# LLNL/ppo_and_friends

Measured on AMD Instinct MI355X. Metric: env_steps_per_sec, higher is better.
Workload: dtype f32; 1 GPU; C2 CartPole-v1 MLP (4->128x3->2 actor, ->1 critic), envs_per_proc=4096, ts_per_rollout=128, fixed-length synthetic trajectories, batch_size=256, epochs_per_iter=10; parallelism=dp1, hip_graphs=True

## Files before the change

### ppo_and_friends_amd/csrc/ppo_update_dev.hpp

```cpp
#pragma once
#include "action_heads.hpp"
#include "wgrad_tile.hpp"
#include <cstddef>
#include <cstring>

namespace ppoaf {

struct WsDev {
    float* hbuf[2];
    float* dbuf[2];
    float* outpart[2];
    float* xbuf[2];
    int W;
    int xcc[2];
    int Bp;
};

struct UpdateDev {
    NetDev net[2];
    const float* params; float* grads; float* exp_avg; float* exp_avg_sq; float* slabs;
    long bucket_total;
    int64_t* step_counts; const float* lr; double* norm_scratch;
    float beta1, beta2, adam_eps, grad_scale, max_norm; int head_kind;
    const float* obs; const float* critic_obs; const void* raw_actions;
    const float* adv; const float* old_lp; const float* rtg; float* values;
    const int64_t* perm; const int32_t* row_map; long n_rows;
    int64_t* cursor; long B, batch_stride, mb_offset, cursor_advance;
    int normalize_values, n_ranks;
    float* vn_mean; float* vn_var; double* vn_count; const double* vn_records;
    const double* adv_records;
    int normalize_adv, use_huber, pregathered;
    float surr_clip, entropy_weight, kl_loss_weight, huber_delta, min_std;
    float* loss_partials; double* totals;
    int n_wg;
    int confine;
    int split;
    WsDev sp;
    int n_slices; int slices[8];
};

inline long ws_seg_off(const NetDev& n) {
    const long szW0 = ((long)n.H * n.in_dim + 3) & ~3L;
    return n.depth == 0 ? 0 : szW0 + n.H + (long)(n.depth - 1) * ((long)n.H * n.H + n.H);
}
inline long ws_seg_len(const NetDev& n) { return n.size - ws_seg_off(n); }

inline int split_wgrad_jobs(const NetDev& n) {
    const int t = n.H / 16, t2 = (t + 1) / 2, p0 = ((n.in_dim + 15) / 16 + 1) / 2;
    return (n.depth - 1) * t * t2 + t * p0 + 1;
}
inline int split_wgrad_per_xcd(const UpdateDev& u) { return (split_wgrad_jobs(u.net[0]) + split_wgrad_jobs(u.net[1]) + 7) / 8; }
inline int split_wgrad_blocks(const UpdateDev& u) { return 8 * split_wgrad_per_xcd(u); }

inline size_t ws_layout(const UpdateDev& u, WsDev* ws, char* base) {
    const long Bp = (u.B + 63) & ~63L;
    size_t off = 0;
    auto take = [&](size_t floats) { const size_t o = off; off += (floats * 4 + 255) & ~(size_t)255; return o; };
    for (int w = 0; w < 2; ++w) {
        const NetDev& n = u.net[w];
        const size_t plane = (size_t)n.depth * Bp * n.H;
        const size_t oh = take(plane), od = take(plane), oo = take((size_t)((u.B + 15) / 16) * ws_seg_len(n));
        const size_t ox = take((size_t)Bp * 64);
        if (ws) {
            ws->hbuf[w] = reinterpret_cast<float*>(base + oh);
            ws->dbuf[w] = reinterpret_cast<float*>(base + od);
            ws->outpart[w] = reinterpret_cast<float*>(base + oo);
            ws->xbuf[w] = reinterpret_cast<float*>(base + ox);
        }
    }
    if (ws) ws->Bp = (int)Bp;
    return off;
}

constexpr int kPairHeaderBytes = 256;
constexpr int kPairRecBytes = 16 * 1024;
constexpr int kPairMaxTiles = 32;
constexpr long long kPairWaitTicks = 200000000LL;

struct PairDev {
    unsigned char* base;
    long net_off[2];
};

inline bool pair_eligible(const NetDev& n) { return n.H == 256 && n.depth >= 2 && n.depth <= 4; }
inline int pair_phases(const NetDev& n) { return 2 * n.depth - 3; }
inline size_t pair_region_offset(const UpdateDev& u) {
    UpdateDev f = u;
    if (u.batch_stride > f.B) f.B = u.batch_stride;
    return ws_layout(f, nullptr, nullptr);
}
inline size_t pair_region_layout(const UpdateDev& u, PairDev* p, char* region) {
    size_t off = kPairHeaderBytes;
    for (int w = 0; w < 2; ++w) {
        const bool on = pair_eligible(u.net[w]);
        if (p) p->net_off[w] = on ? (long)off : 0;
        if (on) off += (size_t)pair_phases(u.net[w]) * kPairMaxTiles * 2 * kPairRecBytes;
    }
    if (p) p->base = reinterpret_cast<unsigned char*>(region);
    return off;
}

constexpr int kWgradThreads = 256;

struct SplitJob {
    int l, ot, itile;
    bool two;
    long ldw;
    long off_w, off_b;
};
template <int H>
__device__ __forceinline__ long split_off_w(const NetDev& nd, const int l) {
    const long szW0 = ((long)H * nd.in_dim + 3) & ~3L;
    return l == 0 ? 0 : szW0 + H + (long)(l - 1) * ((long)H * H + H);
}
template <int H>
__device__ __forceinline__ bool split_job_decode(const UpdateDev& u, const int which, const int job, SplitJob& sj) {
    const auto& nd = u.net[which];
    const int in_dim = nd.in_dim, depth = nd.depth;
    constexpr int t = H / 16, t2 = (t + 1) / 2;
    const int n_it0 = (in_dim + 15) / 16, p0 = (n_it0 + 1) / 2;
    const int n_hidden = (depth - 1) * t * t2, n_l0 = t * p0;
    if (job >= n_hidden + n_l0) return false;
    int n_it;
    if (job < n_hidden) { sj.l = 1 + job / (t * t2); const int jj = job % (t * t2); sj.ot = jj / t2; sj.itile = 2 * (jj % t2); n_it = t; }
    else { sj.l = 0; const int jj = job - n_hidden; sj.ot = jj / p0; sj.itile = 2 * (jj % p0); n_it = n_it0; }
    const int l = sj.l;
    sj.two = sj.itile + 1 < n_it;
    sj.ldw = l >= 1 ? H : in_dim;
    sj.off_w = split_off_w<H>(nd, l);
    sj.off_b = l == 0 ? (((long)H * in_dim + 3) & ~3L)
                      : sj.off_w + (l < depth ? (long)H * H : (((long)nd.out_dim * H + 3) & ~3L));
    return true;
}
template <int H> __device__ __forceinline__ __amdgpu_buffer_rsrc_t split_panel_d(const UpdateDev& u, const int which, const int l) {
    return wgrad_rsrc(u.sp.dbuf[which] + (long)l * ((long)u.sp.Bp * H));
}
template <int H> __device__ __forceinline__ __amdgpu_buffer_rsrc_t split_panel_x(const UpdateDev& u, const int which, const int l) {
    return wgrad_rsrc(l >= 1 ? u.sp.hbuf[which] + (long)(l - 1) * ((long)u.sp.Bp * H) : u.sp.xbuf[which]);
}
__device__ __forceinline__ float split_out_fold(const float* outpart, const int n_hb, const long seg_len, const long idx) {
    float acc = 0.f;
    for (int g0 = 0; g0 < n_hb; g0 += 8) {
        float pv[8];
#pragma unroll
        for (int k = 0; k < 8; ++k) pv[k] = outpart[(long)(g0 + k < n_hb ? g0 + k : 0) * seg_len + idx];
#pragma unroll
        for (int k = 0; k < 8; ++k) if (g0 + k < n_hb) acc += pv[k];
    }
    return acc;
}

__device__ __forceinline__ void ppo_update_bookkeeping_totals(const UpdateDev& u) {
    const int lane = threadIdx.x;
    float p0 = 0.f, p2 = 0.f, p3 = 0.f, p4 = 0.f, p7 = 0.f;
    for (int g = lane; g < u.n_wg; g += 64) {
        const float* a = u.loss_partials + (long)g * 8;
        const float* cc = u.loss_partials + ((long)u.n_wg + g) * 8;
        p0 += a[0]; p3 += a[3]; p4 += a[4]; p7 += a[7]; p2 += cc[2];
    }
    p0 = wave_sum(p0); p2 = wave_sum(p2); p3 = wave_sum(p3); p4 = wave_sum(p4); p7 = wave_sum(p7);
    if (lane == 0) {
        const float n = (float)u.B;
        const float surr = p0 / n, ent = p3 / n, kl = p4 / n, crit = p2 / n;
        float total = surr;
        if (u.entropy_weight != 0.0f) total -= u.entropy_weight * ent;
        if (u.kl_loss_weight > 0.0f) total += u.kl_loss_weight * kl;
        u.totals[0] += (double)surr; u.totals[1] += (double)total; u.totals[2] += (double)crit;
        u.totals[3] += (double)ent; u.totals[4] += (double)kl;
        u.totals[5] += (double)u.loss_partials[5]; u.totals[6] += (double)u.loss_partials[6];
        u.totals[7] += p7 > 0.f ? 1.0 : 0.0;
        u.totals[8] += 1.0;
    }
}
__device__ __forceinline__ void ppo_update_bookkeeping_steps(const UpdateDev& u) {
    const int lane = threadIdx.x;
    if (lane < 2) {
        const int w = lane;
        const int64_t t = u.step_counts[w] + 1;
        u.step_counts[w] = t;
        u.norm_scratch[2 + 2 * w] = 1.0 - pow((double)u.beta1, (double)t);
        u.norm_scratch[3 + 2 * w] = sqrt(1.0 - pow((double)u.beta2, (double)t));
    }
}

__device__ __forceinline__ void ppo_update_bookkeeping_split(const UpdateDev& u) {
    if (threadIdx.x >= 64) return;
    ppo_update_bookkeeping_totals(u);
    ppo_update_bookkeeping_steps(u);
}

int make_update_dev(const ppoaf_ppo_update_args_t* a, UpdateDev& u);

inline ppoaf_ppo_update_args_t copy_update_args(const ppoaf_ppo_update_args_t* args) {
    ppoaf_ppo_update_args_t a;
    std::memset(&a, 0, sizeof(a));
    std::memcpy(&a, args, offsetof(ppoaf_ppo_update_args_t, n_action_slices));
    if (args->head_kind == PPOAF_HEAD_MULTI_CATEGORICAL) {
        a.n_action_slices = args->n_action_slices;
        std::memcpy(a.action_slices, args->action_slices, sizeof(a.action_slices));
    }
    return a;
}

__device__ __forceinline__ unsigned hw_xcc_id() {
    unsigned v;
    asm volatile("s_getreg_b32 %0, hwreg(HW_REG_XCC_ID)" : "=s"(v));
    return v & 0xfu;
}

template <bool NT, typename U>
__device__ __forceinline__ void ppo_head_loss(const U& u, const int which, const int g, const int out_dim,
                                              const float* __restrict__ log_std_p, const int* sRow,
                                              const float* sRowF, const float* sMisc, float* sActF, float* sOut,
                                              float* sDOut, const int lane, const long B) {
    const int s = lane;
    const int row = s < kRows ? sRow[s] : -1;
    const bool live = row >= 0;
    const float inv_B = 1.0f / (float)B;
    float part[8] = {0, 0, 0, 0, 0, 0, 0, 0};
    if (which == 0) {
        float logp = 0.f, ent = 0.f;
        float av = 0.f, lpo = 0.f;
        if (live) {
            av = sRowF[s]; lpo = sRowF[16 + s];
            if (u.normalize_adv) av = (av - sMisc[0]) / (sMisc[1] + 1e-8f);
        }
        if (u.head_kind == PPOAF_HEAD_CATEGORICAL) {
            const int s4 = lane >> 2, q = lane & 3;
            const bool live4 = sRow[s4] >= 0;
            float av4 = 0.f, lpo4 = 0.f;
            if (live4) {
                av4 = sRowF[s4]; lpo4 = sRowF[16 + s4];
                if (u.normalize_adv) av4 = (av4 - sMisc[0]) / (sMisc[1] + 1e-8f);
            }
            auto rsum = [](float v) { return group4_sum(v); };
            auto rmax = [](float v) { return group4_max(v); };
            const int k0 = q, k1 = q + 4;
            const bool v0 = k0 < out_dim, v1 = k1 < out_dim;
            const float z0 = v0 ? sOut[s4 * kMaxOut + k0] : -INFINITY, z1 = v1 ? sOut[s4 * kMaxOut + k1] : -INFINITY;
            const float m = rmax(fmaxf(z0, z1));
            float p0 = v0 ? expf(z0 - m) : 0.f, p1 = v1 ? expf(z1 - m) : 0.f;
            const float inv = 1.0f / rsum(p0 + p1);
            p0 *= inv; p1 *= inv;
            const float s2 = rsum(p0 + p1);
            int a = reinterpret_cast<const int*>(sActF)[s4 * 8];
            a = a < 0 ? 0 : (a >= out_dim ? out_dim - 1 : a);
            const float n0 = p0 / s2, n1 = p1 / s2;
            const float l0 = v0 ? logf(clamp_prob_u(n0)) : 0.f, l1 = v1 ? logf(clamp_prob_u(n1)) : 0.f;
            const float ent4 = -rsum((v0 ? n0 * l0 : 0.f) + (v1 ? n1 * l1 : 0.f));
            const float logp4 = rsum((k0 == a ? l0 : 0.f) + (k1 == a ? l1 : 0.f));
            const float ratio = expf(logp4 - lpo4);
            const float bad4 = (isnan(ratio) || isinf(ratio)) ? 1.f : 0.f;
            const float lo = 1.0f - u.surr_clip, hi = 1.0f + u.surr_clip;
            const float surr1 = ratio * av4, surr2 = fminf(fmaxf(ratio, lo), hi) * av4;
            float glp;
            if (surr1 <= surr2) glp = -av4 * ratio;
            else glp = (ratio >= lo && ratio <= hi) ? -av4 * ratio : 0.f;
            glp *= inv_B;
            const float gH = (u.entropy_weight != 0.0f) ? -u.entropy_weight * inv_B : 0.f;
            auto gk_of = [&](bool valid, int k, float nk, float lg) {
                if (!valid) return 0.f;
                const float ck = clamp_prob_u(nk);
                const float in_range = (nk >= FLT_EPSILON && nk <= 1.0f - FLT_EPSILON) ? 1.f : 0.f;
                float gk = gH * (-lg - nk * in_range / ck);
                if (k == a) gk += glp * in_range / ck;
                return gk;
            };
            float g0 = gk_of(v0, k0, n0, l0), g1 = gk_of(v1, k1, n1, l1);
            const float dot = rsum(g0 * n0 + g1 * n1);
            g0 = (g0 - dot) / s2; g1 = (g1 - dot) / s2;
            const float dot2 = rsum(g0 * p0 + g1 * p1);
            if (live4) {
                if (k0 < 8) sDOut[s4 * kMaxOut + k0] = p0 * (g0 - dot2);
                sDOut[s4 * kMaxOut + k1] = p1 * (g1 - dot2);
            } else {
                sDOut[s4 * kMaxOut + k0] = 0.f; sDOut[s4 * kMaxOut + k1] = 0.f;
                if (q == 0) for (int k2 = 8; k2 < kMaxOut; ++k2) sDOut[s4 * kMaxOut + k2] = 0.f;
            }
            const int src = (lane & 15) * 4;
            const float r_surr = __shfl(-fminf(surr1, surr2), src, 64), r_ent = __shfl(ent4, src, 64);
            const float r_kl = __shfl(lpo4 - logp4, src, 64), r_bad = __shfl(bad4, src, 64);
            if (live) { part[0] = r_surr; part[3] = r_ent; part[4] = r_kl; part[7] = r_bad; }
        } else if (u.head_kind >= PPOAF_HEAD_MULTI_CATEGORICAL) {
            if (live) {
                float z[8], dz[8];
#pragma unroll
                for (int k = 0; k < 8; ++k) z[k] = k < out_dim ? sOut[s * kMaxOut + k] : 0.f;
                const bool mcat = u.head_kind == PPOAF_HEAD_MULTI_CATEGORICAL;
                const float* x = sActF + s * 8;
                float p[8], sm[8];
                unsigned first = 0u, pick = 0u;
                if (mcat) {
                    first = mcat_starts(u.n_slices, u.slices);
                    mcat_probs(z, first, out_dim, p, sm);
                    pick = mcat_pick(reinterpret_cast<const int*>(x), u.n_slices, u.slices);
                    logp = mcat_logp(p, sm, pick);
                } else {
                    logp = bern_logp(z, x, out_dim);
                }
                const float ratio = expf(logp - lpo);
                if (isnan(ratio) || isinf(ratio)) part[7] = 1.f;
                const float lo = 1.0f - u.surr_clip, hi = 1.0f + u.surr_clip;
                const float surr1 = ratio * av, surr2 = fminf(fmaxf(ratio, lo), hi) * av;
                float glp;
                if (surr1 <= surr2) glp = -av * ratio;
                else glp = (ratio >= lo && ratio <= hi) ? -av * ratio : 0.f;
                glp *= inv_B;
                const float gH = (u.entropy_weight != 0.0f) ? -u.entropy_weight * inv_B : 0.f;
                ent = mcat ? mcat_entropy_grad(p, sm, first, pick, out_dim, glp, gH, dz)
                           : bern_entropy_grad(z, x, out_dim, glp, gH, dz);
                part[0] = -fminf(surr1, surr2);
                part[3] = ent;
                part[4] = lpo - logp;
#pragma unroll
                for (int k = 0; k < 8; ++k) sDOut[s * kMaxOut + k] = dz[k];
            } else if (s < kRows) {
                for (int k = 0; k < kMaxOut; ++k) sDOut[s * kMaxOut + k] = 0.f;
            }
        } else if (live) {
            const float* log_std = log_std_p;
            const float* x = sActF + s * 8;
            float lp = 0.f, slog = 0.f;
            ent = 0.f;
            for (int d = 0; d < out_dim; ++d) {
                const float sd = fmaxf(softplus_u(ld1<NT>(log_std + d)), u.min_std);
                const float mu = sOut[s * kMaxOut + d];
                const float zz = x[d] - mu;
                const float l0 = -logf(sd) - 0.91893853320467274178f;
                float l = -(zz * zz) / (2.0f * sd * sd) + l0;
                l = fminf(fmaxf(l, -100.f), 100.f);
                lp += l;
                const float th = tanhf(x[d]);
                slog += logf(fmaxf(1.0f - th * th, 1e-6f));
                const float thm = tanhf(mu);
                ent += logf(fmaxf(1.0f - thm * thm, 1e-6f)) - fminf(fmaxf(l0, -100.f), 100.f);
            }
            logp = lp - slog;
            const float ratio = expf(logp - lpo);
            if (isnan(ratio) || isinf(ratio)) part[7] = 1.f;
            const float lo = 1.0f - u.surr_clip, hi = 1.0f + u.surr_clip;
            const float surr1 = ratio * av, surr2 = fminf(fmaxf(ratio, lo), hi) * av;
            part[0] = -fminf(surr1, surr2);
            part[3] = ent;
            part[4] = lpo - logp;
            float glp;
            if (surr1 <= surr2) glp = -av * ratio;
            else glp = (ratio >= lo && ratio <= hi) ? -av * ratio : 0.f;
            glp *= inv_B;
            const float gH = (u.entropy_weight != 0.0f) ? -u.entropy_weight * inv_B : 0.f;
            for (int d = 0; d < out_dim; ++d) {
                const float ls = ld1<NT>(log_std + d);
                const float sp = softplus_u(ls), sd = fmaxf(sp, u.min_std);
                const float mu = sOut[s * kMaxOut + d];
                const float zz = x[d] - mu;
                const float l0 = -logf(sd) - 0.91893853320467274178f;
                const float l = -(zz * zz) / (2.0f * sd * sd) + l0;
                const float pass = (l >= -100.f && l <= 100.f) ? 1.f : 0.f;
                const float pass0 = (l0 >= -100.f && l0 <= 100.f) ? 1.f : 0.f;
                const float thm = tanhf(mu);
                const float pass_t = (1.0f - thm * thm >= 1e-6f) ? 1.f : 0.f;
                sDOut[s * kMaxOut + d] = glp * pass * zz / (sd * sd) - gH * pass_t * 2.0f * thm;
                if (d == 0) for (int k2 = out_dim; k2 < 8; ++k2) sDOut[s * kMaxOut + k2] = 0.f;
                const float dmax = sp > u.min_std ? 1.f : (sp == u.min_std ? 0.5f : 0.f);
                const float dsp = ls > 20.f ? 1.f : 1.0f / (1.0f + expf(-ls));
                sOut[s * kMaxOut + 8 + d] = (glp * pass * (zz * zz / (sd * sd * sd) - 1.0f / sd) + gH * pass0 / sd) * dmax * dsp;
            }
        } else if (s < kRows) {
            for (int k = 0; k < kMaxOut; ++k) sDOut[s * kMaxOut + k] = 0.f;
            if (u.head_kind == PPOAF_HEAD_GAUSSIAN)
                for (int d = 0; d < 8; ++d) sOut[s * kMaxOut + 8 + d] = 0.f;
        }
    } else {
        if (live) {
            const float v = sOut[s * kMaxOut];
            float rt = sRowF[32 + s];
            if (u.normalize_values) rt = (rt - sMisc[2]) / sqrtf(sMisc[3] + 1e-8f);
            const float diff = v - rt;
            float l, dl;
            if (u.use_huber) {
                const float ad = fabsf(diff);
                if (ad < u.huber_delta) { l = 0.5f * diff * diff; dl = diff; }
                else { l = u.huber_delta * (ad - 0.5f * u.huber_delta); dl = diff > 0.f ? u.huber_delta : -u.huber_delta; }
            } else { l = diff * diff; dl = 2.0f * diff; }
            part[2] = l;
            sDOut[s * kMaxOut] = dl * inv_B;
            for (int k2 = 1; k2 < 8; ++k2) sDOut[s * kMaxOut + k2] = 0.f;
            u.values[row] = v;
        } else if (s < kRows) {
            for (int k2 = 0; k2 < 8; ++k2) sDOut[s * kMaxOut + k2] = 0.f;
        }
    }
#pragma unroll
    for (int k = 0; k < 8; ++k) {
        float v = (lane < kRows) ? part[k] : 0.f;
        v = group16_sum(v);
        part[k] = v;
    }
    if (lane == 0) {
        if (which == 0 && g == 0) { part[5] = sMisc[0]; part[6] = sMisc[1]; }
        float* lp = u.loss_partials + ((long)which * u.n_wg + g) * 8;
#pragma unroll
        for (int k = 0; k < 8; ++k) lp[k] = part[k];
    }
}

}
```

### ppo_and_friends_amd/csrc/ppo_update_rowtile.hpp

```cpp
#pragma once
#include "ppo_update_dev.hpp"

namespace ppoaf {

extern __shared__ __attribute__((aligned(16))) unsigned char ppo_update_smem[];

#ifdef PPOAF_STAMPS
#ifndef PPOAF_STAMP_BLOCK
#define PPOAF_STAMP_BLOCK 0
#endif
static __device__ unsigned long long g_ppo_update_stamps[2][16];
#define PPOAF_STAMP(k)                                                                   \
    do {                                                                                 \
        if (blockIdx.x == PPOAF_STAMP_BLOCK && threadIdx.x == 0) {                       \
            unsigned long long t_;                                                       \
            asm volatile("s_memtime %0\n\ts_waitcnt lgkmcnt(0)" : "=s"(t_)::"memory");    \
            g_ppo_update_stamps[0][k] = t_;                                              \
        }                                                                                \
    } while (0)
#else
#define PPOAF_STAMP(k) do {} while (0)
#endif



template <int HT, bool NT>
__device__ __forceinline__ void load_fwd_set(const float* __restrict__ W, int n0, int lane, float4 (&fr)[HT]) {
    if constexpr (NT) load_fwd_frags<HT, true>(W, n0, lane, fr);
    else load_fwd_lines_buf<HT>(W, n0, lane, fr);
}
template <int HT, bool NT>
__device__ __forceinline__ f32x4 mfma_fwd_set(const float* __restrict__ A, int HS, int lane, const float4 (&fr)[HT], float init,
                                              float* __restrict__ scratch) {
    if constexpr (NT) return mfma_rows_x_frags<HT>(A, HS, lane, fr, init);
    else return mfma_rows_x_lines<HT>(A, HS, lane, fr, init, scratch);
}

__device__ __forceinline__ int rowtile_request_args(const UpdateDev& u, int b) {
    const NetDev& a = u.net[0];
    const NetDev& c = u.net[1];
    asm("" : "+s"(b)
        : "s"(a.in_dim), "s"(a.H), "s"(a.depth), "s"(a.out_dim), "s"(a.act), "s"((&a.act)[1]), "s"(a.offset), "s"(a.size), "s"(a.log_std_off),
          "s"(c.in_dim), "s"(c.H), "s"(c.depth), "s"(c.out_dim), "s"(c.act), "s"((&c.act)[1]), "s"(c.offset), "s"(c.size), "s"(c.log_std_off),
          "s"(u.params), "s"(u.norm_scratch), "s"(u.head_kind),
          "s"(u.obs), "s"(u.critic_obs), "s"(u.raw_actions), "s"(u.adv), "s"(u.old_lp), "s"(u.rtg), "s"(u.values), "s"(u.perm),
          "s"(u.row_map), "s"(u.n_rows), "s"(u.cursor), "s"(u.B), "s"(u.batch_stride), "s"(u.mb_offset), "s"(u.cursor_advance),
          "s"(u.normalize_values), "s"(u.n_ranks), "s"(u.vn_mean), "s"(u.vn_var), "s"(u.vn_count), "s"(u.vn_records),
          "s"(u.adv_records), "s"(u.normalize_adv), "s"(u.use_huber), "s"(u.pregathered), "s"(u.surr_clip),
          "s"(u.n_wg), "s"(u.confine));
    const long cur = u.cursor[0];
    asm("" : "+s"(b)
        : "s"(cur), "s"(u.entropy_weight), "s"(u.kl_loss_weight), "s"(u.huber_delta), "s"(u.min_std), "s"(u.loss_partials),
          "s"(u.sp.hbuf[0]), "s"(u.sp.hbuf[1]), "s"(u.sp.dbuf[0]), "s"(u.sp.dbuf[1]), "s"(u.sp.outpart[0]), "s"(u.sp.outpart[1]),
          "s"(u.sp.xbuf[0]), "s"(u.sp.xbuf[1]), "s"(u.sp.W), "s"(u.sp.xcc[0]), "s"(u.sp.xcc[1]), "s"(u.sp.Bp), "s"(u.n_slices),
          "s"(u.slices[0]), "s"(u.slices[1]), "s"(u.slices[2]), "s"(u.slices[3]), "s"(u.slices[4]), "s"(u.slices[5]),
          "s"(u.slices[6]), "s"(u.slices[7]));
    return b;
}

template <int HT, bool SPLIT, bool TABLES>
__device__ __forceinline__ void ppo_update_fwd_bwd_body_as(const UpdateDev& u, const int which, const int g) {
    constexpr bool NT = false;
    constexpr long mb_extra = 0;
    constexpr int H = 16 * HT, HS = H + 4;
    int tid_ = threadIdx.x;
    if (NT) {
        asm volatile("" : "+v"(tid_));
        __builtin_assume(tid_ >= 0 && tid_ < kThreadsU);
    }
    const int tid = tid_, lane = tid & 63, wave = NT ? __builtin_amdgcn_readfirstlane(tid >> 6) : (tid >> 6);
    const auto& nd = u.net[which];
    const int in_dim = nd.in_dim, depth = nd.depth, out_dim = nd.out_dim, act = nd.act;
    const int NT0 = (in_dim + 15) >> 4;
    const int INP = 16 * NT0 + 4;
    const float* P = u.params + nd.offset;
    const long B = u.B;
    const long mb = u.cursor[0] + u.mb_offset + mb_extra;
    const long base = mb * u.batch_stride;
    const long szW0 = ((long)H * in_dim + 3) & ~3L;
    auto offW = [&](int l) -> long { return l == 0 ? 0 : szW0 + H + (long)(l - 1) * (H * H + H); };
    auto offB = [&](int l) -> long {
        return l == 0 ? szW0 : offW(l) + (l < depth ? (long)H * H : (((long)out_dim * H + 3) & ~3L));
    };
    float* slab = SPLIT ? u.sp.outpart[which] + (long)g * (nd.size - offW(depth)) - offW(depth)
                        : u.slabs + (long)g * u.bucket_total + nd.offset;
    auto publish_rows = [&](const float* src, float* panel) {
        float* dst = panel + (long)g * kRows * H;
        for (int i = tid; i < kRows * (H / 4); i += kThreadsU) {
            const int r = i / (H / 4), c4 = i - r * (H / 4);
            *reinterpret_cast<float4*>(dst + (long)r * H + 4 * c4) = *reinterpret_cast<const float4*>(src + r * HS + 4 * c4);
        }
    };
    const long sp_plane = SPLIT ? (long)u.sp.Bp * H : 0;

    PPOAF_STAMP(0);
    int zl = 0;
    if (NT) asm volatile("" : "+s"(zl));
    float* smem = reinterpret_cast<float*>(ppo_update_smem + zl);
    int* sRow = reinterpret_cast<int*>(smem);
    float* sMisc = smem + 16;
    float* sRowF = smem + 32;
    float* sActF = smem + 80;
    float* sBias = smem + 208;
    float* sWout = sBias + (depth + 1) * H;
    float* sX = sWout + 8 * H;
    float* sH = sX + kRows * INP;
    float* sD0 = sH + (long)depth * kRows * HS;
    float* sD1 = sD0 + kRows * HS;
    float* sOut = sD1 + kRows * HS;
    float* sDOut = sOut + kRows * kMaxOut;
    float* sScr = sDOut + kRows * kMaxOut + wave * 2 * kLineSlot;

    if (!NT && g == 0 && which == 0 && tid == 0) { u.norm_scratch[0] = 0.0; u.norm_scratch[1] = 0.0; }

    const bool has_tile = HT >= kNW || wave < HT;
    static_assert(!TABLES || HT <= kNW, "deep prefetch: one output tile per wave");
    const bool deep = TABLES || (depth == 3 && HT <= kNW);
    float4 fr[HT], fr2[HT];
    const bool l0_pre = in_dim <= 16 && HT <= kNW && has_tile;
    float l0w[4] = {0.f, 0.f, 0.f, 0.f};
    float l2_touch = 0.f;
    constexpr int kCopyRegs = 4;
    float bias_reg[kCopyRegs], wout_reg[kCopyRegs];
    const int n_bias = (depth + 1) * H, n_wout = out_dim * H;
    const bool copy_fits = n_bias <= kCopyRegs * kThreadsU && n_wout <= kCopyRegs * kThreadsU;
    auto request_weights = [&]() {
        if (NT && deep && has_tile) {
            load_fwd_set<HT, NT>(P + offW(1), wave * 16, lane, fr);
            load_fwd_set<HT, NT>(P + offW(2), wave * 16, lane, fr2);
        }
        if (l0_pre) {
            const float* w = P + offW(0) + (long)(wave * 16 + (lane & 15)) * in_dim;
#pragma unroll
            for (int j = 0; j < 4; ++j) { const int k = 4 * j + (lane >> 4); if (k < in_dim) l0w[j] = ld1<NT>(w + k); }
        }
#ifndef PPOAF_L2_TOUCH_MAX_HT
#define PPOAF_L2_TOUCH_MAX_HT 8
#endif
        if (!deep && !NT && HT <= PPOAF_L2_TOUCH_MAX_HT) for (long i = (long)tid * 32; i < nd.size; i += (long)kThreadsU * 32) l2_touch += P[i];
        if (copy_fits) {
#pragma unroll
            for (int r = 0; r < kCopyRegs; ++r) {
                const int i = tid + r * kThreadsU;
                bias_reg[r] = 0.f; wout_reg[r] = 0.f;
                if (i < n_bias) { const int l = i / H, j = i - l * H; if (l < depth || j < out_dim) bias_reg[r] = ld1<NT>(P + offB(l) + j); }
                if (i < n_wout) wout_reg[r] = ld1<NT>(P + offW(depth) + i);
            }
        }
    };
    auto request_hidden_sets = [&]() {
        if (!NT && deep && has_tile) {
            load_fwd_set<HT, NT>(P + offW(1), wave * 16, lane, fr);
            load_fwd_set<HT, NT>(P + offW(2), wave * 16, lane, fr2);
        }
    };
    const float* x_src = which == 0 ? u.obs : u.critic_obs;
    const bool x_pre = !NT && (TABLES || u.pregathered) && kRows * in_dim <= 2 * kThreadsU;
    float xr[2] = {0.f, 0.f};
    if (x_pre) {
#pragma unroll
        for (int q = 0; q < 2; ++q) {
            const int idx = tid + q * kThreadsU;
            if (idx < kRows * in_dim && (long)g * kRows + idx / in_dim < B) xr[q] = x_src[(base + (long)g * kRows) * in_dim + idx];
        }
    }
    if constexpr (TABLES) asm volatile("; ppoaf_rowtile_tables_prologue");
    if (!NT) request_weights();

    constexpr int kActRegs = 8;
    constexpr int kVnPre = 2;
    const bool row_lane = tid < kRows && (long)g * kRows + tid < B;
    static_assert(!TABLES || !NT, "per-epoch tables: separate launches only");
    constexpr bool early = TABLES;
    const int n_act = which != 0 ? 0 : u.head_kind == PPOAF_HEAD_CATEGORICAL ? 1
                    : u.head_kind == PPOAF_HEAD_MULTI_CATEGORICAL ? u.n_slices : out_dim;
    long perm_v = -1;
    float av = 0.f, lpo = 0.f, rt = 0.f;
    int act_bits[kActRegs];
#pragma unroll
    for (int j = 0; j < kActRegs; ++j) act_bits[j] = 0;
    auto request_row_scalars = [&](const long di) {
        if (which == 0) {
            av = u.adv[di]; lpo = u.old_lp[di];
            if (u.head_kind == PPOAF_HEAD_CATEGORICAL) {
                act_bits[0] = (int)reinterpret_cast<const int64_t*>(u.raw_actions)[di];
            } else if (u.head_kind == PPOAF_HEAD_MULTI_CATEGORICAL) {
#pragma unroll
                for (int j = 0; j < kActRegs; ++j)
                    if (j < n_act) act_bits[j] = (int)reinterpret_cast<const int64_t*>(u.raw_actions)[(long)di * u.n_slices + j];
            } else {
#pragma unroll
                for (int d = 0; d < kActRegs; ++d)
                    if (d < n_act) act_bits[d] = __float_as_int(reinterpret_cast<const float*>(u.raw_actions)[(long)di * out_dim + d]);
            }
        } else {
            rt = u.rtg[di];
        }
    };
    if (row_lane) {
        const long s = (long)g * kRows + tid;
        perm_v = u.perm[base + s];
        if (early) request_row_scalars(base + s);
    }
    const bool stat_lane = tid == 64;
    double adv_rec[3] = {0.0, 0.0, 0.0}, vn_rec[kVnPre][3];
    float vn_m = 0.f, vn_v = 0.f;
    double vn_cnt = 0.0;
#pragma unroll
    for (int r = 0; r < kVnPre; ++r) { vn_rec[r][0] = 0.0; vn_rec[r][1] = 0.0; vn_rec[r][2] = 0.0; }
    if (stat_lane) {
        if (which == 0) {
            if (u.normalize_adv) {
                const double* rec = u.adv_records + mb * 3;
                adv_rec[0] = rec[0]; adv_rec[1] = rec[1]; adv_rec[2] = rec[2];
            }
        } else {
            const int slot = (int)(mb & 1);
            vn_m = ld1<NT>(u.vn_mean + slot); vn_v = ld1<NT>(u.vn_var + slot);
            vn_cnt = ld1<NT>(u.vn_count + slot);
            if (u.normalize_values) {
#pragma unroll
                for (int r = 0; r < kVnPre; ++r) {
                    if (r < u.n_ranks) {
                        const double* rec = u.vn_records + (mb * u.n_ranks + r) * 3;
                        vn_rec[r][0] = rec[0]; vn_rec[r][1] = rec[1]; vn_rec[r][2] = rec[2];
                    }
                }
            }
        }
    }
    double vn_n = 0.0, vn_bm = 0.0, vn_M2 = 0.0;
    auto vn_merge = [&](const double nb, const double mean, const double m2) {
        if (nb <= 0.0) return;
        const double d = mean - vn_bm, nn = vn_n + nb;
        vn_bm += d * (nb / nn);
        vn_M2 += m2 + d * d * vn_n * nb / nn;
        vn_n = nn;
    };
    if (stat_lane && which != 0 && u.normalize_values && u.n_ranks > kVnPre) {
#pragma unroll
        for (int r = 0; r < kVnPre; ++r) vn_merge(vn_rec[r][0], vn_rec[r][1], vn_rec[r][2]);
        for (int r = kVnPre; r < u.n_ranks; ++r) {
            const double* rec = u.vn_records + (mb * u.n_ranks + r) * 3;
            vn_merge(rec[0], rec[1], rec[2]);
        }
    }
    if (!NT) request_hidden_sets();

    if (tid < kRows) {
        auto store_row = [&](const int row, const bool have) {
            if (have) {
#pragma unroll
                for (int j = 0; j < kActRegs; ++j)
                    if (j < n_act) reinterpret_cast<int*>(sActF)[tid * 8 + j] = act_bits[j];
            }
            sRow[tid] = row;
            sRowF[tid] = av; sRowF[16 + tid] = lpo; sRowF[32 + tid] = rt;
        };
        if constexpr (TABLES) {
            int row = -1;
            if (row_lane && perm_v >= 0 && perm_v < u.n_rows) row = (int)perm_v;
            store_row(row, row_lane);
        } else {
            int row = -1;
            long di = -1;
            if (row_lane) {
                const long p = perm_v;
                if (p >= 0 && p < u.n_rows) row = u.row_map ? u.row_map[p] : (int)p;
                di = u.pregathered ? base + (long)g * kRows + tid : row;
            }
            if (di >= 0 && !early) request_row_scalars(di);
            store_row(row, di >= 0);
        }
    }

    if (stat_lane) {
        if (which == 0) {
            float mean_f = 0.f, std_f = 1.f;
            if (u.normalize_adv) {
                mean_f = (float)adv_rec[1];
                std_f = (float)sqrt(adv_rec[2] / (adv_rec[0] - 1.0));
            }
            sMisc[0] = mean_f; sMisc[1] = std_f;
        } else {
            const int slot = (int)(mb & 1);
            float m = vn_m, v = vn_v;
            double cnt = vn_cnt;
            if (u.normalize_values) {
                if (u.n_ranks <= kVnPre) {
#pragma unroll
                    for (int r = 0; r < kVnPre; ++r)
                        if (r < u.n_ranks) vn_merge(vn_rec[r][0], vn_rec[r][1], vn_rec[r][2]);
                }
                const double n = vn_n, bm = vn_bm, M2 = vn_M2;
                if (n > 0.0) {
                    const float batch_mean = (float)bm, batch_var = (float)(M2 / n);
                    const float delta = batch_mean - m;
                    const double new_count = cnt + n;
                    const float new_mean = (float)((double)m + (double)delta * (n / new_count));
                    const double m_2 = (double)v * cnt + (double)batch_var * n +
                                       (double)(delta * delta) * cnt * n / (cnt + n);
                    m = new_mean; v = (float)(m_2 / (cnt + n)); cnt = new_count;
                }
            }
            sMisc[2] = m; sMisc[3] = v;
            if (g == 0) { u.vn_mean[slot ^ 1] = m; u.vn_var[slot ^ 1] = v; u.vn_count[slot ^ 1] = cnt; }
        }
    }
    if (copy_fits) {
#pragma unroll
        for (int r = 0; r < kCopyRegs; ++r) {
            const int i = tid + r * kThreadsU;
            if (i < n_bias) sBias[i] = bias_reg[r];
            if (i < n_wout) sWout[i] = wout_reg[r];
        }
    } else {
        for (int l = 0; l <= depth; ++l) {
            const int n = (l == depth) ? out_dim : H;
            const float* bb = P + offB(l);
            for (int i = tid; i < n; i += kThreadsU) sBias[l * H + i] = ld1<NT>(bb + i);
        }
        for (int i = tid; i < out_dim * H; i += kThreadsU) sWout[i] = ld1<NT>(P + offW(depth) + i);
    }
    for (int i = tid; i < kRows * INP; i += kThreadsU) sX[i] = 0.f;
    __syncthreads();
    PPOAF_STAMP(1);

    if (x_pre) {
#pragma unroll
        for (int q = 0; q < 2; ++q) {
            const int idx = tid + q * kThreadsU;
            const int s = idx / in_dim, i = idx - s * in_dim;
            if (idx < kRows * in_dim && sRow[s] >= 0) sX[s * INP + i] = xr[q];
        }
    } else {
        const float* src = x_src;
        for (int idx = tid; idx < kRows * in_dim; idx += kThreadsU) {
            const int s = idx / in_dim, i = idx - s * in_dim;
            const int row = sRow[s];
            const long di = (TABLES || u.pregathered) ? base + (long)g * kRows + s : row;
            if (row >= 0) sX[s * INP + i] = src[di * in_dim + i];
        }
    }
    if (!deep && depth > 1 && has_tile) load_fwd_set<HT, NT>(P + offW(1), wave * 16, lane, fr);
    __syncthreads();
    PPOAF_STAMP(2);
    if (SPLIT) {
        float* xb = u.sp.xbuf[which] + (long)g * kRows * 64;
        for (int i = tid; i < kRows * 64; i += kThreadsU) {
            const int r = i >> 6, c = i & 63;
            xb[i] = c < 16 * NT0 ? sX[r * INP + c] : 0.f;
        }
    }

    for (int nt = wave; nt < HT; nt += kNW) {
        const int o = nt * 16 + (lane & 15);
        const float bv = sBias[o];
        f32x4 acc = {bv, bv, bv, bv};
        const float* w = P + offW(0) + (long)o * in_dim;
        const float* arow = sX + (lane & 15) * INP;
        for (int k0 = 0; k0 < in_dim; k0 += 16) {
            float bq[4];
#pragma unroll
            for (int j = 0; j < 4; ++j) {
                const int k = k0 + 4 * j + (lane >> 4);
                bq[j] = l0_pre ? l0w[j] : (k < in_dim ? ld1<NT>(w + k) : 0.f);
            }
#pragma unroll
            for (int j = 0; j < 4; ++j)
                acc = __builtin_amdgcn_mfma_f32_16x16x4f32(arow[k0 + 4 * j + (lane >> 4)], bq[j], acc, 0, 0, 0);
        }
#pragma unroll
        for (int r = 0; r < 4; ++r) sH[(4 * (lane >> 4) + r) * HS + o] = act_fwd(acc[r], act);
    }
    __syncthreads();
    PPOAF_STAMP(3);

    for (int l = 1; l < depth; ++l) {
        const float* Hp = sH + (long)(l - 1) * kRows * HS;
        float* Hc = sH + (long)l * kRows * HS;
        if (SPLIT) publish_rows(Hp, u.sp.hbuf[which] + (long)(l - 1) * sp_plane);
        for (int nt = wave; nt < HT; nt += kNW) {
            const int o = nt * 16 + (lane & 15);
            f32x4 acc;
            if (deep) {
                if (l == 1) {
                    acc = mfma_fwd_set<HT, NT>(Hp, HS, lane, fr, sBias[l * H + o], sScr);
                    load_dgrad_frags<HT, NT>(P + offW(2), wave * 16, lane, fr);
                } else {
                    acc = mfma_fwd_set<HT, NT>(Hp, HS, lane, fr2, sBias[l * H + o], sScr);
                    load_dgrad_frags<HT, NT>(P + offW(1), wave * 16, lane, fr2);
                }
            } else {
            if (nt != wave) load_fwd_set<HT, NT>(P + offW(l), nt * 16, lane, fr);
            acc = mfma_fwd_set<HT, NT>(Hp, HS, lane, fr, sBias[l * H + o], sScr);
            if (nt + kNW >= HT) {
                if (l + 1 < depth) load_fwd_set<HT, NT>(P + offW(l + 1), wave * 16, lane, fr);
                else load_dgrad_frags<HT, NT>(P + offW(l), wave * 16, lane, fr);
            }
            }
#pragma unroll
            for (int r = 0; r < 4; ++r) Hc[(4 * (lane >> 4) + r) * HS + o] = act_fwd(acc[r], act);
            
        }
        __syncthreads();
        
    }
    PPOAF_STAMP(4);
    const float* Hlast = sH + (long)(depth - 1) * kRows * HS;

    if (tid < 256) {
        const int s = tid >> 4, part = tid & 15;
        for (int k = 0; k < out_dim; ++k) {
            float acc = 0.f;
#pragma unroll
            for (int i = 0; i < HT; ++i) acc = fmaf(Hlast[s * HS + part + 16 * i], sWout[k * H + part + 16 * i], acc);
            acc = group16_sum(acc);
            if (part == 0) sOut[s * kMaxOut + k] = acc + sBias[depth * H + k];
        }
    }
    __syncthreads();
    PPOAF_STAMP(5);

    if (wave == 0) {
        ppo_head_loss<NT>(u, which, g, out_dim, P + nd.log_std_off, sRow, sRowF, sMisc, sActF, sOut, sDOut, lane, B);
    }
    __syncthreads();
    PPOAF_STAMP(6);

    {
        if (tid < H) {
            const int i = tid;
            float h[kRows];
#pragma unroll
            for (int s = 0; s < kRows; ++s) h[s] = Hlast[s * HS + i];
            for (int k = 0; k < out_dim; ++k) {
                float d[kRows];
#pragma unroll
                for (int s = 0; s < kRows; ++s) d[s] = sDOut[s * kMaxOut + k];
                float acc = 0.f;
#pragma unroll
                for (int s = 0; s < kRows; ++s) acc = fmaf(d[s], h[s], acc);
                slab[offW(depth) + (long)k * H + i] = acc;
            }
        }
        const int out_pad = SPLIT ? ((out_dim + 3) & ~3) : out_dim;
        if (tid >= 256 && tid < 256 + out_pad) {
            const int k = tid - 256;
            float acc = 0.f;
            if (k < out_dim) {
#pragma unroll
                for (int s = 0; s < kRows; ++s) acc += sDOut[s * kMaxOut + k];
            }
            slab[offB(depth) + k] = acc;
        }
        if (which == 0 && u.head_kind == PPOAF_HEAD_GAUSSIAN && tid >= 320 && tid < 320 + out_pad) {
            const int d = tid - 320;
            float acc = 0.f;
            if (d < out_dim) {
#pragma unroll
                for (int s = 0; s < kRows; ++s) acc += sOut[s * kMaxOut + 8 + d];
            }
            slab[nd.log_std_off + d] = acc;
        }
        if (tid >= 256) {
            const int t2 = tid - 256;
            const int s = t2 >> 4, ig = t2 & 15;
            float d[8];
            const float4 d0 = *reinterpret_cast<const float4*>(sDOut + s * kMaxOut);
            const float4 d1 = *reinterpret_cast<const float4*>(sDOut + s * kMaxOut + 4);
            d[0] = d0.x; d[1] = d0.y; d[2] = d0.z; d[3] = d0.w; d[4] = d1.x; d[5] = d1.y; d[6] = d1.z; d[7] = d1.w;
            float hv[HT], acc[HT];
#pragma unroll
            for (int ii = 0; ii < HT; ++ii) { hv[ii] = Hlast[s * HS + ig + 16 * ii]; acc[ii] = 0.f; }
#pragma unroll
            for (int k = 0; k < 8; ++k) {
                if (k < out_dim) {
#pragma unroll
                    for (int ii = 0; ii < HT; ++ii) acc[ii] = fmaf(d[k], sWout[k * H + ig + 16 * ii], acc[ii]);
                }
            }
#pragma unroll
            for (int ii = 0; ii < HT; ++ii) sD0[s * HS + ig + 16 * ii] = acc[ii] * act_bwd(hv[ii], act);
        }
    }
    __syncthreads();
    PPOAF_STAMP(7);

    float* Dc = sD0;
    float* Dn = sD1;
    for (int l = depth - 1; l >= 1; --l) {
        const float* Hin = sH + (long)(l - 1) * kRows * HS;
        if (SPLIT) publish_rows(Dc, u.sp.dbuf[which] + (long)l * sp_plane);
        for (int nt = wave; nt < HT; nt += kNW) {
            f32x4 acc;
            if (deep) {
                acc = l == 2 ? mfma_rows_x_frags<HT>(Dc, HS, lane, fr, 0.f) : mfma_rows_x_frags<HT>(Dc, HS, lane, fr2, 0.f);
            } else {
            if (nt != wave) load_dgrad_frags<HT, NT>(P + offW(l), nt * 16, lane, fr);
            acc = mfma_rows_x_frags<HT>(Dc, HS, lane, fr, 0.f);
            if (nt + kNW >= HT && l - 1 >= 1) load_dgrad_frags<HT, NT>(P + offW(l - 1), wave * 16, lane, fr);
            }
#pragma unroll
            for (int r = 0; r < 4; ++r) {
                const int s = 4 * (lane >> 4) + r, i = nt * 16 + (lane & 15);
                Dn[s * HS + i] = acc[r] * act_bwd(Hin[s * HS + i], act);
            }
        }
        if (l == depth - 1) PPOAF_STAMP(10);
        if (!SPLIT) {
            for (int mt = wave; mt < HT; mt += kNW) {
                if (HT <= 8) wgrad_mtile_full<(HT <= 8 ? HT : 1)>(Dc, HS, Hin, HS, mt * 16, lane, slab + offW(l), H);
                else wgrad_mtile(Dc, HS, Hin, HS, mt * 16, HT, H, lane, slab + offW(l), H);
            }
            if (l == depth - 1) PPOAF_STAMP(11);
            for (int o = tid; o < H; o += kThreadsU) {
                float acc = 0.f;
#pragma unroll
                for (int s = 0; s < kRows; ++s) acc += Dc[s * HS + o];
                slab[offB(l) + o] = acc;
            }
        }
        if (l == depth - 1) PPOAF_STAMP(12);
        __syncthreads();
        if (l == depth - 1) PPOAF_STAMP(13);
        float* t = Dc; Dc = Dn; Dn = t;
    }
    PPOAF_STAMP(8);

    if (SPLIT) {
        publish_rows(Dc, u.sp.dbuf[which]);
    } else {
        for (int mt = wave; mt < HT; mt += kNW)
            wgrad_mtile(Dc, HS, sX, INP, mt * 16, NT0, in_dim, lane, slab + offW(0), in_dim);
        for (int o = tid; o < H; o += kThreadsU) {
            float acc = 0.f;
#pragma unroll
            for (int s = 0; s < kRows; ++s) acc += Dc[s * HS + o];
            slab[offB(0) + o] = acc;
        }
    }
    if (l2_touch == 1.2345e38f) u.loss_partials[0] = l2_touch;
    PPOAF_STAMP(9);
}

template <int HT, bool SPLIT = false>
__device__ __forceinline__ void ppo_update_fwd_bwd_body(const UpdateDev& u, const int which, const int g) {
    if constexpr (HT <= kNW) {
        if (u.net[which].depth == 3 && u.pregathered && !u.row_map) {
            ppo_update_fwd_bwd_body_as<HT, SPLIT, true>(u, which, g);
            return;
        }
    }
    ppo_update_fwd_bwd_body_as<HT, SPLIT, false>(u, which, g);
}

constexpr size_t kRowtileLineFloats = (size_t)kNW * 2 * kLineSlot;
inline size_t rowtile_lds_floats(const NetDev& n) {
    const size_t HS = n.H + 4, INP = 16 * ((n.in_dim + 15) / 16) + 4;
    return 208 + (size_t)(n.depth + 1) * n.H + 8 * (size_t)n.H + kRows * INP + (size_t)n.depth * kRows * HS + 2 * kRows * HS +
           2 * kRows * kMaxOut;
}

}
```

Baseline: 1.135 million env-steps/s.

## Defer head reductions and output-layer wgrad off the critical path in rowtile update

The head loss is split into per-row work, a value store, and a block reduction. The cross-lane reduction and the loss-partial and value writes are moved to idle waves at the end of the kernel, with per-row partials stashed in LDS. The output-layer weight and bias gradients also move to the end. The last-layer dgrad is spread across all threads with vectorized LDS reads, and split-mode panel publishing is staged through registers so the global stores can be issued after the MFMA loop. Together these shorten the serial head-to-backward section, at the cost of more registers and extra LDS traffic.

After: 1.175 million env-steps/s, median of 6. +3.5%, better.

```diff
diff --git a/ppo_and_friends_amd/csrc/ppo_update_dev.hpp b/ppo_and_friends_amd/csrc/ppo_update_dev.hpp
--- a/ppo_and_friends_amd/csrc/ppo_update_dev.hpp
+++ b/ppo_and_friends_amd/csrc/ppo_update_dev.hpp
@@ -5,6 +5,26 @@
 #include <cstring>
 
 namespace ppoaf {
+
+#ifdef PPOAF_STAMPS
+#ifndef PPOAF_STAMP_BLOCK
+#define PPOAF_STAMP_BLOCK 0
+#endif
+static __device__ unsigned long long g_ppo_update_stamps[2][16];
+#define PPOAF_STAMP_AT(row, k, t0)                                                       \
+    do {                                                                                 \
+        if (blockIdx.x == PPOAF_STAMP_BLOCK && threadIdx.x == (t0)) {                    \
+            unsigned long long t_;                                                       \
+            asm volatile("s_memtime %0\n\ts_waitcnt lgkmcnt(0)" : "=s"(t_)::"memory");    \
+            g_ppo_update_stamps[row][k] = t_;                                            \
+        }                                                                                \
+    } while (0)
+#define PPOAF_STAMP(k) PPOAF_STAMP_AT(0, k, 0)
+#define PPOAF_STAMP_W(k, w) PPOAF_STAMP_AT(1, k, 64 * (w))
+#else
+#define PPOAF_STAMP(k) do {} while (0)
+#define PPOAF_STAMP_W(k, w) do {} while (0)
+#endif
 
 struct WsDev {
     float* hbuf[2];
@@ -209,7 +229,7 @@
 }
 
 template <bool NT, typename U>
-__device__ __forceinline__ void ppo_head_loss(const U& u, const int which, const int g, const int out_dim,
+__device__ __forceinline__ void ppo_head_rows(const U& u, const int which, const int out_dim,
                                               const float* __restrict__ log_std_p, const int* sRow,
                                               const float* sRowF, const float* sMisc, float* sActF, float* sOut,
                                               float* sDOut, const int lane, const long B) {
@@ -277,10 +297,7 @@
                 sDOut[s4 * kMaxOut + k0] = 0.f; sDOut[s4 * kMaxOut + k1] = 0.f;
                 if (q == 0) for (int k2 = 8; k2 < kMaxOut; ++k2) sDOut[s4 * kMaxOut + k2] = 0.f;
             }
-            const int src = (lane & 15) * 4;
-            const float r_surr = __shfl(-fminf(surr1, surr2), src, 64), r_ent = __shfl(ent4, src, 64);
-            const float r_kl = __shfl(lpo4 - logp4, src, 64), r_bad = __shfl(bad4, src, 64);
-            if (live) { part[0] = r_surr; part[3] = r_ent; part[4] = r_kl; part[7] = r_bad; }
+            if (live4) { part[0] = -fminf(surr1, surr2); part[3] = ent4; part[4] = lpo4 - logp4; part[7] = bad4; }
         } else if (u.head_kind >= PPOAF_HEAD_MULTI_CATEGORICAL) {
             if (live) {
                 float z[8], dz[8];
@@ -385,17 +402,37 @@
             part[2] = l;
             sDOut[s * kMaxOut] = dl * inv_B;
             for (int k2 = 1; k2 < 8; ++k2) sDOut[s * kMaxOut + k2] = 0.f;
-            u.values[row] = v;
         } else if (s < kRows) {
             for (int k2 = 0; k2 < 8; ++k2) sDOut[s * kMaxOut + k2] = 0.f;
         }
     }
-#pragma unroll
-    for (int k = 0; k < 8; ++k) {
-        float v = (lane < kRows) ? part[k] : 0.f;
-        v = group16_sum(v);
-        part[k] = v;
-    }
+    asm volatile("" ::: "memory");
+    const bool cat = which == 0 && u.head_kind == PPOAF_HEAD_CATEGORICAL;
+    const int prow = cat ? (lane >> 2) : s;
+    if (cat ? (lane & 3) == 0 : s < kRows) {
+        float* pk = sActF + prow * 8;
+        pk[0] = part[0]; pk[2] = part[2]; pk[3] = part[3]; pk[4] = part[4]; pk[7] = part[7];
+    }
+}
+
+template <typename U>
+__device__ __forceinline__ void ppo_head_values(const U& u, const int* sRow, const float* sOut, const int lane) {
+    if (lane < kRows) {
+        const int row = sRow[lane];
+        if (row >= 0) u.values[row] = sOut[lane * kMaxOut];
+    }
+}
+
+template <typename U>
+__device__ __forceinline__ void ppo_head_block(const U& u, const int which, const int g, const float* sMisc,
+                                               const float* sActF, const int lane) {
+    float part[8] = {0, 0, 0, 0, 0, 0, 0, 0};
+    if (lane < kRows) {
+        const float* pk = sActF + lane * 8;
+        part[0] = pk[0]; part[2] = pk[2]; part[3] = pk[3]; part[4] = pk[4]; part[7] = pk[7];
+    }
+#pragma unroll
+    for (int k = 0; k < 8; ++k) part[k] = group16_sum(part[k]);
     if (lane == 0) {
         if (which == 0 && g == 0) { part[5] = sMisc[0]; part[6] = sMisc[1]; }
         float* lp = u.loss_partials + ((long)which * u.n_wg + g) * 8;
@@ -404,4 +441,14 @@
     }
 }
 
-}
+template <bool NT, typename U>
+__device__ __forceinline__ void ppo_head_loss(const U& u, const int which, const int g, const int out_dim,
+                                              const float* __restrict__ log_std_p, const int* sRow,
+                                              const float* sRowF, const float* sMisc, float* sActF, float* sOut,
+                                              float* sDOut, const int lane, const long B) {
+    ppo_head_rows<NT>(u, which, out_dim, log_std_p, sRow, sRowF, sMisc, sActF, sOut, sDOut, lane, B);
+    if (which != 0) ppo_head_values(u, sRow, sOut, lane);
+    ppo_head_block(u, which, g, sMisc, sActF, lane);
+}
+
+}
diff --git a/ppo_and_friends_amd/csrc/ppo_update_rowtile.hpp b/ppo_and_friends_amd/csrc/ppo_update_rowtile.hpp
--- a/ppo_and_friends_amd/csrc/ppo_update_rowtile.hpp
+++ b/ppo_and_friends_amd/csrc/ppo_update_rowtile.hpp
@@ -4,23 +4,6 @@
 namespace ppoaf {
 
 extern __shared__ __attribute__((aligned(16))) unsigned char ppo_update_smem[];
-
-#ifdef PPOAF_STAMPS
-#ifndef PPOAF_STAMP_BLOCK
-#define PPOAF_STAMP_BLOCK 0
-#endif
-static __device__ unsigned long long g_ppo_update_stamps[2][16];
-#define PPOAF_STAMP(k)                                                                   \
-    do {                                                                                 \
-        if (blockIdx.x == PPOAF_STAMP_BLOCK && threadIdx.x == 0) {                       \
-            unsigned long long t_;                                                       \
-            asm volatile("s_memtime %0\n\ts_waitcnt lgkmcnt(0)" : "=s"(t_)::"memory");    \
-            g_ppo_update_stamps[0][k] = t_;                                              \
-        }                                                                                \
-    } while (0)
-#else
-#define PPOAF_STAMP(k) do {} while (0)
-#endif
 
 
 
@@ -58,6 +41,28 @@
     return b;
 }
 
+template <int CP> __device__ __forceinline__ void lds_read_adjacent(const float* p, float (&v)[CP]) {
+    if constexpr (CP % 4 == 0) {
+#pragma unroll
+        for (int q = 0; q < CP / 4; ++q) {
+            const float4 t = *reinterpret_cast<const float4*>(p + 4 * q);
+            v[4 * q] = t.x; v[4 * q + 1] = t.y; v[4 * q + 2] = t.z; v[4 * q + 3] = t.w;
+        }
+    } else {
+#pragma unroll
+        for (int q = 0; q < CP; ++q) v[q] = p[q];
+    }
+}
+template <int CP> __device__ __forceinline__ void lds_write_adjacent(float* p, const float (&v)[CP]) {
+    if constexpr (CP % 4 == 0) {
+#pragma unroll
+        for (int q = 0; q < CP / 4; ++q) *reinterpret_cast<float4*>(p + 4 * q) = make_float4(v[4 * q], v[4 * q + 1], v[4 * q + 2], v[4 * q + 3]);
+    } else {
+#pragma unroll
+        for (int q = 0; q < CP; ++q) p[q] = v[q];
+    }
+}
+
 template <int HT, bool SPLIT, bool TABLES>
 __device__ __forceinline__ void ppo_update_fwd_bwd_body_as(const UpdateDev& u, const int which, const int g) {
     constexpr bool NT = false;
@@ -84,12 +89,30 @@
     };
     float* slab = SPLIT ? u.sp.outpart[which] + (long)g * (nd.size - offW(depth)) - offW(depth)
                         : u.slabs + (long)g * u.bucket_total + nd.offset;
-    auto publish_rows = [&](const float* src, float* panel) {
+    constexpr int kPub = (kRows * (H / 4) + kThreadsU - 1) / kThreadsU;
+    constexpr bool kPubLate = HT <= kNW;
+    float4 pub[kPub];
+    auto publish_read = [&](const float* src) {
+#pragma unroll
+        for (int q = 0; q < kPub; ++q) {
+            const int i = tid + q * kThreadsU, r = i / (H / 4), c4 = i - r * (H / 4);
+            if (i < kRows * (H / 4)) pub[q] = *reinterpret_cast<const float4*>(src + r * HS + 4 * c4);
+        }
+    };
+    auto publish_store = [&](float* panel) {
         float* dst = panel + (long)g * kRows * H;
-        for (int i = tid; i < kRows * (H / 4); i += kThreadsU) {
-            const int r = i / (H / 4), c4 = i - r * (H / 4);
-            *reinterpret_cast<float4*>(dst + (long)r * H + 4 * c4) = *reinterpret_cast<const float4*>(src + r * HS + 4 * c4);
-        }
+#pragma unroll
+        for (int q = 0; q < kPub; ++q) {
+            const int i = tid + q * kThreadsU, r = i / (H / 4), c4 = i - r * (H / 4);
+            if (i < kRows * (H / 4)) *reinterpret_cast<float4*>(dst + (long)r * H + 4 * c4) = pub[q];
+        }
+    };
+    auto publish_begin = [&](const float* src, float* panel) {
+        publish_read(src);
+        if constexpr (!kPubLate) publish_store(panel);
+    };
+    auto publish_end = [&](float* panel) {
+        if constexpr (kPubLate) { __builtin_amdgcn_sched_barrier(0); publish_store(panel); }
     };
     const long sp_plane = SPLIT ? (long)u.sp.Bp * H : 0;
 
@@ -379,7 +402,7 @@
     for (int l = 1; l < depth; ++l) {
         const float* Hp = sH + (long)(l - 1) * kRows * HS;
         float* Hc = sH + (long)l * kRows * HS;
-        if (SPLIT) publish_rows(Hp, u.sp.hbuf[which] + (long)(l - 1) * sp_plane);
+        if (SPLIT) publish_begin(Hp, u.sp.hbuf[which] + (long)(l - 1) * sp_plane);
         for (int nt = wave; nt < HT; nt += kNW) {
             const int o = nt * 16 + (lane & 15);
             f32x4 acc;
@@ -401,10 +424,9 @@
             }
 #pragma unroll
             for (int r = 0; r < 4; ++r) Hc[(4 * (lane >> 4) + r) * HS + o] = act_fwd(acc[r], act);
-            
-        }
+        }
+        if (SPLIT) publish_end(u.sp.hbuf[which] + (long)(l - 1) * sp_plane);
         __syncthreads();
-        
     }
     PPOAF_STAMP(4);
     const float* Hlast = sH + (long)(depth - 1) * kRows * HS;
@@ -423,67 +445,41 @@
     PPOAF_STAMP(5);
 
     if (wave == 0) {
-        ppo_head_loss<NT>(u, which, g, out_dim, P + nd.log_std_off, sRow, sRowF, sMisc, sActF, sOut, sDOut, lane, B);
+        if constexpr (TABLES) asm volatile("; ppoaf_rowtile_head_rows_begin");
+        ppo_head_rows<NT>(u, which, out_dim, P + nd.log_std_off, sRow, sRowF, sMisc, sActF, sOut, sDOut, lane, B);
+        if constexpr (TABLES) asm volatile("; ppoaf_rowtile_head_rows_end");
+        PPOAF_STAMP_W(0, 0);
     }
     __syncthreads();
+    if constexpr (TABLES) asm volatile("; ppoaf_rowtile_middle_begin");
     PPOAF_STAMP(6);
 
     {
-        if (tid < H) {
-            const int i = tid;
-            float h[kRows];
-#pragma unroll
-            for (int s = 0; s < kRows; ++s) h[s] = Hlast[s * HS + i];
-            for (int k = 0; k < out_dim; ++k) {
-                float d[kRows];
-#pragma unroll
-                for (int s = 0; s < kRows; ++s) d[s] = sDOut[s * kMaxOut + k];
-                float acc = 0.f;
-#pragma unroll
-                for (int s = 0; s < kRows; ++s) acc = fmaf(d[s], h[s], acc);
-                slab[offW(depth) + (long)k * H + i] = acc;
-            }
-        }
-        const int out_pad = SPLIT ? ((out_dim + 3) & ~3) : out_dim;
-        if (tid >= 256 && tid < 256 + out_pad) {
-            const int k = tid - 256;
-            float acc = 0.f;
+        constexpr int CP = H / 32;
+        static_assert(kThreadsU == 32 * kRows && H % 32 == 0, "dz_last: 32 lane groups per row");
+        const int s = tid >> 5, c0 = (tid & 31) * CP;
+        float d[8];
+        const float4 d0 = *reinterpret_cast<const float4*>(sDOut + s * kMaxOut);
+        const float4 d1 = *reinterpret_cast<const float4*>(sDOut + s * kMaxOut + 4);
+        d[0] = d0.x; d[1] = d0.y; d[2] = d0.z; d[3] = d0.w; d[4] = d1.x; d[5] = d1.y; d[6] = d1.z; d[7] = d1.w;
+        float hv[CP], acc[CP], wv[CP];
+        lds_read_adjacent<CP>(Hlast + s * HS + c0, hv);
+#pragma unroll
+        for (int ii = 0; ii < CP; ++ii) acc[ii] = 0.f;
+#pragma unroll
+        for (int k = 0; k < 8; ++k) {
             if (k < out_dim) {
-#pragma unroll
-                for (int s = 0; s < kRows; ++s) acc += sDOut[s * kMaxOut + k];
-            }
-            slab[offB(depth) + k] = acc;
-        }
-        if (which == 0 && u.head_kind == PPOAF_HEAD_GAUSSIAN && tid >= 320 && tid < 320 + out_pad) {
-            const int d = tid - 320;
-            float acc = 0.f;
-            if (d < out_dim) {
-#pragma unroll
-                for (int s = 0; s < kRows; ++s) acc += sOut[s * kMaxOut + 8 + d];
-            }
-            slab[nd.log_std_off + d] = acc;
-        }
-        if (tid >= 256) {
-            const int t2 = tid - 256;
-            const int s = t2 >> 4, ig = t2 & 15;
-            float d[8];
-            const float4 d0 = *reinterpret_cast<const float4*>(sDOut + s * kMaxOut);
-            const float4 d1 = *reinterpret_cast<const float4*>(sDOut + s * kMaxOut + 4);
-            d[0] = d0.x; d[1] = d0.y; d[2] = d0.z; d[3] = d0.w; d[4] = d1.x; d[5] = d1.y; d[6] = d1.z; d[7] = d1.w;
-            float hv[HT], acc[HT];
-#pragma unroll
-            for (int ii = 0; ii < HT; ++ii) { hv[ii] = Hlast[s * HS + ig + 16 * ii]; acc[ii] = 0.f; }
-#pragma unroll
-            for (int k = 0; k < 8; ++k) {
-                if (k < out_dim) {
-#pragma unroll
-                    for (int ii = 0; ii < HT; ++ii) acc[ii] = fmaf(d[k], sWout[k * H + ig + 16 * ii], acc[ii]);
-                }
-            }
-#pragma unroll
-            for (int ii = 0; ii < HT; ++ii) sD0[s * HS + ig + 16 * ii] = acc[ii] * act_bwd(hv[ii], act);
-        }
-    }
+                lds_read_adjacent<CP>(sWout + k * H + c0, wv);
+#pragma unroll
+                for (int ii = 0; ii < CP; ++ii) acc[ii] = fmaf(d[k], wv[ii], acc[ii]);
+            }
+        }
+#pragma unroll
+        for (int ii = 0; ii < CP; ++ii) acc[ii] = acc[ii] * act_bwd(hv[ii], act);
+        lds_write_adjacent<CP>(sD0 + s * HS + c0, acc);
+    }
+    PPOAF_STAMP_W(2, 0); PPOAF_STAMP_W(3, 4); PPOAF_STAMP_W(4, 5);
+    if constexpr (TABLES) asm volatile("; ppoaf_rowtile_middle_end");
     __syncthreads();
     PPOAF_STAMP(7);
 
@@ -491,7 +487,7 @@
     float* Dn = sD1;
     for (int l = depth - 1; l >= 1; --l) {
         const float* Hin = sH + (long)(l - 1) * kRows * HS;
-        if (SPLIT) publish_rows(Dc, u.sp.dbuf[which] + (long)l * sp_plane);
+        if (SPLIT) publish_begin(Dc, u.sp.dbuf[which] + (long)l * sp_plane);
         for (int nt = wave; nt < HT; nt += kNW) {
             f32x4 acc;
             if (deep) {
@@ -507,6 +503,7 @@
                 Dn[s * HS + i] = acc[r] * act_bwd(Hin[s * HS + i], act);
             }
         }
+        if (SPLIT) publish_end(u.sp.dbuf[which] + (long)l * sp_plane);
         if (l == depth - 1) PPOAF_STAMP(10);
         if (!SPLIT) {
             for (int mt = wave; mt < HT; mt += kNW) {
@@ -529,7 +526,8 @@
     PPOAF_STAMP(8);
 
     if (SPLIT) {
-        publish_rows(Dc, u.sp.dbuf[which]);
+        publish_read(Dc);
+        publish_store(u.sp.dbuf[which]);
     } else {
         for (int mt = wave; mt < HT; mt += kNW)
             wgrad_mtile(Dc, HS, sX, INP, mt * 16, NT0, in_dim, lane, slab + offW(0), in_dim);
@@ -539,6 +537,47 @@
             for (int s = 0; s < kRows; ++s) acc += Dc[s * HS + o];
             slab[offB(0) + o] = acc;
         }
+    }
+    PPOAF_STAMP_W(6, 0);
+
+    if (tid < H) {
+        const int i = tid;
+        float h[kRows];
+#pragma unroll
+        for (int s = 0; s < kRows; ++s) h[s] = Hlast[s * HS + i];
+        for (int k = 0; k < out_dim; ++k) {
+            float d[kRows];
+#pragma unroll
+            for (int s = 0; s < kRows; ++s) d[s] = sDOut[s * kMaxOut + k];
+            float acc = 0.f;
+#pragma unroll
+            for (int s = 0; s < kRows; ++s) acc = fmaf(d[s], h[s], acc);
+            slab[offW(depth) + (long)k * H + i] = acc;
+        }
+    }
+    {
+        const int out_pad = SPLIT ? ((out_dim + 3) & ~3) : out_dim;
+        if (tid >= 256 && tid < 256 + out_pad) {
+            const int k = tid - 256;
+            float acc = 0.f;
+            if (k < out_dim) {
+#pragma unroll
+                for (int s = 0; s < kRows; ++s) acc += sDOut[s * kMaxOut + k];
+            }
+            slab[offB(depth) + k] = acc;
+        }
+        if (which == 0 && u.head_kind == PPOAF_HEAD_GAUSSIAN && tid >= 320 && tid < 320 + out_pad) {
+            const int d = tid - 320;
+            float acc = 0.f;
+            if (d < out_dim) {
+#pragma unroll
+                for (int s = 0; s < kRows; ++s) acc += sOut[s * kMaxOut + 8 + d];
+            }
+            slab[nd.log_std_off + d] = acc;
+        }
+        if (which != 0 && wave == 6) ppo_head_values(u, sRow, sOut, lane);
+        if (wave == 7) ppo_head_block(u, which, g, sMisc, sActF, lane);
+        PPOAF_STAMP_W(5, 0); PPOAF_STAMP_W(1, 7);
     }
     if (l2_touch == 1.2345e38f) u.loss_partials[0] = l2_touch;
     PPOAF_STAMP(9);
```
